# little-little-point-cloud-group/buildingSegment

Hardware: AMD Instinct MI355X
Metric: Mpoints/s segmented (kNN+normal+label) (higher is better)
Workload: dtype int32 coordinates / f64 normals; 1 GPU; urban_50m; points_per_gpu=50000000, k=16, max_nn=50, rg_mode=0, largest_plane=135921, seed_attempts=6951, fallback_queries=0, rg_rounds=25, validation_rejects=6, tie_rows=971975, parallelism=1 GPU, whole path

## Files before the change

### buildingsegment_amd/csrc/bs_knn.hip

```cpp
#include <cstdlib>
#include <type_traits>

#include "bs_common.h"
#include "bs_normal.h"

namespace bs {

namespace {

constexpr int BS_FAST_RINGS = 2;
constexpr int BS_GENERAL_RINGS = 6;

template <bool TILED>
using GridOf = std::conditional_t<TILED, TiledGridDev, GridDev>;

template <bool TILED>
__device__ inline uint64_t cell_key(uint32_t cx, uint32_t cy, uint32_t cz, uint64_t kbase)
{
  if constexpr (TILED)
    return kbase | morton_cell(cx, cy, cz);
  else
    return pack_cell(cx, cy, cz);
}

__device__ inline void tile_enter(TiledGridDev& g, int64_t s, uint64_t& kbase, int64_t& lo, int64_t& hi)
{
  const int32_t t = tile_of(g.tile_off, g.n_tiles, s);
  const TileDesc d = g.tiles[t];
#pragma unroll
  for (int a = 0; a < 3; a++) {
    g.mn[a] = d.mn[a];
    g.dim[a] = d.dim[a];
  }
  kbase = (uint64_t)t << g.mbits;
  lo = g.tile_off[t];
  hi = g.tile_off[t + 1];
}

template <bool TILED = false>
__device__ inline bool cell_lookup(const GridDev& g, uint32_t cx, uint32_t cy, uint32_t cz, int& start,
                                   int& end, uint64_t kbase = 0)
{
  const uint64_t k = cell_key<TILED>(cx, cy, cz, kbase);
  uint32_t h = hash_cell(k) & g.hmask;
  for (;;) {
    const int4 raw = *reinterpret_cast<const int4*>(&g.table[h]);
    const uint64_t ek = (uint64_t)(uint32_t)raw.x | ((uint64_t)(uint32_t)raw.y << 32);
    if (ek == k) {
      start = raw.z;
      end = raw.w;
      return true;
    }
    if (ek == ~0ull)
      return false;
    h = (h + 1) & g.hmask;
  }
}

__device__ inline bool guaranteed_radius(const GridDev& g, const int q[3], const int ci[3], int rho,
                                         uint64_t& R2)
{
  uint32_t R = 0xFFFFFFFFu;
  bool bounded = false;
#pragma unroll
  for (int a = 0; a < 3; a++) {
    if (ci[a] - rho > 0) {
      int lo = g.mn[a] + (ci[a] - rho) * g.cell;
      R = min(R, (uint32_t)(q[a] - lo + 1));
      bounded = true;
    }
    if (ci[a] + rho < g.dim[a] - 1) {
      int hi = g.mn[a] + (ci[a] + rho + 1) * g.cell - 1;
      R = min(R, (uint32_t)(hi + 1 - q[a]));
      bounded = true;
    }
  }
  R2 = (uint64_t)R * (uint64_t)R;
  return bounded;
}

__device__ inline void moments_add(Moments& m, int x, int y, int z)
{
  m.sx += x;
  m.sy += y;
  m.sz += z;
  m.sxx += (uint64_t)((int64_t)x * x);
  m.syy += (uint64_t)((int64_t)y * y);
  m.szz += (uint64_t)((int64_t)z * z);
  m.sxy += (int64_t)x * y;
  m.sxz += (int64_t)x * z;
  m.syz += (int64_t)y * z;
  m.n += 1;
}

template <int KC, bool TILED = false>
__global__ __launch_bounds__(256) void knn_fast_kernel(GridOf<TILED> g, int64_t q_begin, int64_t q_end, int K,
                                                       int max_nn, double r2, int32_t* __restrict__ neigh,
                                                       double* __restrict__ normals,
                                                       int32_t* __restrict__ fb_list,
                                                       int32_t* __restrict__ fb_count, uint64_t cert_r2,
                                                       unsigned long long* __restrict__ uncert,
                                                       int32_t* __restrict__ npos, unsigned long long* __restrict__ tie_rows)
{
  const int64_t s = xcd_logical_block() * (int64_t)blockDim.x + threadIdx.x;
  if (s >= g.n)
    return;
  const int32_t loc = g.slocal[s];
  if (loc < q_begin || loc >= q_end)
    return;
  uint64_t kbase = 0;
  if constexpr (TILED) {
    int64_t lo, hi;
    tile_enter(g, s, kbase, lo, hi);
  }
  uint64_t runner = ~0ull;
  const int4 P = g.spts[s];
  const int q[3] = {P.x, P.y, P.z};
  const int ci[3] = {(int)((uint32_t)(P.x - g.mn[0]) / (uint32_t)g.cell),
                     (int)((uint32_t)(P.y - g.mn[1]) / (uint32_t)g.cell),
                     (int)((uint32_t)(P.z - g.mn[2]) / (uint32_t)g.cell)};
  uint64_t best[KC];
  int bpos[KC];
#pragma unroll
  for (int j = 0; j < KC; j++) {
    best[j] = ~0ull;
    bpos[j] = 0;
  }
  Moments m = {};
  bool done = false;
  for (int rho = 0; rho <= BS_FAST_RINGS && !done; rho++) {
    for (int dz = -rho; dz <= rho; dz++) {
      const int cz = ci[2] + dz;
      if (cz < 0 || cz >= g.dim[2])
        continue;
      for (int dy = -rho; dy <= rho; dy++) {
        const int cy = ci[1] + dy;
        if (cy < 0 || cy >= g.dim[1])
          continue;
        const bool face = (dz == -rho || dz == rho || dy == -rho || dy == rho);
        const int step = face ? 1 : (rho > 0 ? 2 * rho : 1);
        for (int dx = -rho; dx <= rho; dx += step) {
          const int cx = ci[0] + dx;
          if (cx < 0 || cx >= g.dim[0])
            continue;
          int cs, ce;
          if (!cell_lookup<TILED>(g, (uint32_t)cx, (uint32_t)cy, (uint32_t)cz, cs, ce, kbase))
            continue;
          for (int t = cs; t < ce; t++) {
            const int4 c = g.spts[t];
            const int ex = c.x - q[0], ey = c.y - q[1], ez = c.z - q[2];
            const uint32_t d2 = (uint32_t)(ex * ex) + (uint32_t)(ey * ey) + (uint32_t)(ez * ez);
            uint64_t key = ((uint64_t)d2 << 32) | (uint32_t)c.w;
            if (key < best[KC - 1]) {
              int pay = t;
#pragma unroll
              for (int j = 0; j < KC; j++) {
                const bool lt = key < best[j];
                const uint64_t hi = lt ? best[j] : key;
                const int ph = lt ? bpos[j] : pay;
                best[j] = lt ? key : best[j];
                bpos[j] = lt ? pay : bpos[j];
                key = hi;
                pay = ph;
              }
            }
            runner = key < runner ? key : runner;
            if ((double)d2 < r2)
              moments_add(m, c.x, c.y, c.z);
          }
        }
      }
    }
    uint64_t R2;
    const bool bounded = guaranteed_radius(g, q, ci, rho, R2);
    if (!bounded) {
      done = true;
    } else {
      uint64_t kth = ~0ull;
#pragma unroll
      for (int j = 0; j < KC; j++)
        kth = (j == K - 1) ? best[j] : kth;
      const bool knn_ok = kth != ~0ull && (kth >> 32) < R2;
      const bool nrm_ok = (double)R2 >= r2;
      done = knn_ok && nrm_ok;
    }
  }
  uint64_t kth_final = ~0ull;
#pragma unroll
  for (int j = 0; j < KC; j++)
    kth_final = (j == K - 1) ? best[j] : kth_final;
  if (!done || m.n > max_nn || kth_final == ~0ull) {
    const int slot = atomicAdd(fb_count, 1);
    fb_list[slot] = (int32_t)s;
    return;
  }
  int32_t* row = neigh + (int64_t)(loc - q_begin) * K;
#pragma unroll
  for (int j = 0; j < KC; j++)
    if (j < K)
      row[j] = (int32_t)(uint32_t)best[j];
  if (npos) {
    int32_t* prow = npos + s * K;
#pragma unroll
    for (int j = 0; j < KC; j++)
      if (j < K)
        prow[j] = bpos[j];
  }
  if (normals) {
    const V3 nv = normal_from_moments(m);
    double* o = normals + 3 * (int64_t)(loc - q_begin);
    o[0] = nv.x;
    o[1] = nv.y;
    o[2] = nv.z;
    if (npos) {
      double* po = pnorm_of(npos, g.n, K) + 3 * s;
      po[0] = nv.x;
      po[1] = nv.y;
      po[2] = nv.z;
    }
  }
  if (cert_r2 && (kth_final >> 32) >= cert_r2)
    atomicAdd(uncert, 1ull);
  if (tie_rows) {
    bool tie = false;
    uint64_t next = runner;
#pragma unroll
    for (int j = 0; j + 1 < KC; j++) {
      tie = tie || (j + 1 < K && (best[j] >> 32) == (best[j + 1] >> 32));
      next = (j + 1 == K) ? best[j + 1] : next;
    }
    tie = tie || (next != ~0ull && (next >> 32) == (kth_final >> 32));
    if (tie)
      atomicAdd(tie_rows, 1ull);
  }
}

#ifndef BS_KNN_CAP4
#define BS_KNN_CAP4 0
#endif
constexpr int KBUF = 8;

template <int KC, bool REL32, bool TILED = false>
__global__ __launch_bounds__(256) __attribute__((amdgpu_waves_per_eu(KC == 16 && REL32 && BS_KNN_CAP4 ? 4 : 2))) void knn_fast2_kernel(GridOf<TILED> g, int64_t q_begin, int64_t q_end, int K,
                                                       int max_nn, double r2, int32_t* __restrict__ neigh,
                                                       double* __restrict__ normals,
                                                       int32_t* __restrict__ fb_list,
                                                       int32_t* __restrict__ fb_count, uint64_t cert_r2,
                                                       unsigned long long* __restrict__ uncert,
                                                       int32_t* __restrict__ npos, unsigned long long* __restrict__ tie_rows)
{
  const int64_t s = xcd_logical_block() * (int64_t)blockDim.x + threadIdx.x;
  if (s >= g.n)
    return;
  const int32_t loc = g.slocal[s];
  if (loc < q_begin || loc >= q_end)
    return;
  uint64_t kbase = 0;
  if constexpr (TILED) {
    int64_t lo, hi;
    tile_enter(g, s, kbase, lo, hi);
  }
  uint64_t runner = ~0ull;
  const int4 P = g.spts[s];
  const int q[3] = {P.x, P.y, P.z};
  const int ci[3] = {(int)((uint32_t)(P.x - g.mn[0]) / (uint32_t)g.cell),
                     (int)((uint32_t)(P.y - g.mn[1]) / (uint32_t)g.cell),
                     (int)((uint32_t)(P.z - g.mn[2]) / (uint32_t)g.cell)};
  __shared__ uint32_t blo[KBUF][256], bhi[KBUF][256];
  __shared__ int bps[KBUF][256];
  int nbuf = 0;
  uint64_t best[KC];
  int bpos[KC];
#pragma unroll
  for (int j = 0; j < KC; j++) {
    best[j] = ~0ull;
    bpos[j] = 0;
  }
  Moments m = {};
  int rsx = 0, rsy = 0, rsz = 0, rsxx = 0, rsyy = 0, rszz = 0, rsxy = 0, rsxz = 0, rsyz = 0, rn = 0;
  bool done = false;
  auto flush = [&]() {
    uint64_t bk[KBUF];
    int bp[KBUF];
#pragma unroll
    for (int i = 0; i < KBUF; i++) {
      const bool have = i < nbuf;
      bk[i] = have ? (((uint64_t)bhi[i][threadIdx.x] << 32) | blo[i][threadIdx.x]) : ~0ull;
      bp[i] = have ? bps[i][threadIdx.x] : 0;
    }
    nbuf = 0;
#define BS_CE(ka, pa, kb, pb)            \
  do {                                   \
    const bool sw_ = (kb) < (ka);        \
    const uint64_t tk_ = (ka);           \
    const int tp_ = (pa);                \
    (ka) = sw_ ? (kb) : (ka);            \
    (pa) = sw_ ? (pb) : (pa);            \
    (kb) = sw_ ? tk_ : (kb);             \
    (pb) = sw_ ? tp_ : (pb);             \
  } while (0)
    constexpr int net[19][2] = {{0, 1}, {2, 3}, {4, 5}, {6, 7}, {0, 2}, {1, 3}, {4, 6}, {5, 7}, {1, 2}, {5, 6},
                                {0, 4}, {3, 7}, {1, 5}, {2, 6}, {1, 4}, {3, 6}, {2, 4}, {3, 5}, {3, 4}};
#pragma unroll
    for (int c = 0; c < 19; c++)
      BS_CE(bk[net[c][0]], bp[net[c][0]], bk[net[c][1]], bp[net[c][1]]);
#pragma unroll
    for (int i = 0; i < KBUF; i++)
      BS_CE(best[KC - KBUF + i], bpos[KC - KBUF + i], bk[KBUF - 1 - i], bp[KBUF - 1 - i]);
#pragma unroll
    for (int i = 0; i < KBUF; i++)
      runner = bk[i] < runner ? bk[i] : runner;
#pragma unroll
    for (int d = KC / 2; d >= 1; d >>= 1) {
#pragma unroll
      for (int i = 0; i < KC; i++)
        if ((i & d) == 0)
          BS_CE(best[i], bpos[i], best[i + d], bpos[i + d]);
    }
#undef BS_CE
  };
  for (int rho = 0; rho <= BS_FAST_RINGS && !done; rho++) {
    for (int dz = -rho; dz <= rho; dz++) {
      const int cz = ci[2] + dz;
      if (cz < 0 || cz >= g.dim[2])
        continue;
      for (int dy = -rho; dy <= rho; dy++) {
        const int cy = ci[1] + dy;
        if (cy < 0 || cy >= g.dim[1])
          continue;
        const bool face = (dz == -rho || dz == rho || dy == -rho || dy == rho);
        const int step = face ? 1 : (rho > 0 ? 2 * rho : 1);
        for (int dx0 = -rho; dx0 <= rho; dx0 += 3 * step) {
          int4 raw[3];
          uint64_t ck[3];
          uint32_t hh[3];
          bool want[3];
#pragma unroll
          for (int u = 0; u < 3; u++) {
            const int dx = dx0 + u * step;
            const int cx = ci[0] + dx;
            want[u] = dx <= rho && cx >= 0 && cx < g.dim[0];
            ck[u] = cell_key<TILED>((uint32_t)(want[u] ? cx : ci[0]), (uint32_t)cy, (uint32_t)cz, kbase);
            hh[u] = hash_cell(ck[u]) & g.hmask;
            raw[u] = *reinterpret_cast<const int4*>(&g.table[hh[u]]);
          }
          int cs3[3], ce3[3];
#pragma unroll
          for (int u = 0; u < 3; u++) {
            cs3[u] = 0;
            ce3[u] = 0;
            if (!want[u])
              continue;
            for (;;) {
              const uint64_t ek = (uint64_t)(uint32_t)raw[u].x | ((uint64_t)(uint32_t)raw[u].y << 32);
              if (ek == ck[u]) {
                cs3[u] = raw[u].z;
                ce3[u] = raw[u].w;
                break;
              }
              if (ek == ~0ull)
                break;
              hh[u] = (hh[u] + 1) & g.hmask;
              raw[u] = *reinterpret_cast<const int4*>(&g.table[hh[u]]);
            }
          }
#pragma unroll 1
          for (int u = 0; u < 3; u++) {
            const int cs = u == 0 ? cs3[0] : (u == 1 ? cs3[1] : cs3[2]);
            const int ce = u == 0 ? ce3[0] : (u == 1 ? ce3[1] : ce3[2]);
            for (int t0 = cs; t0 < ce; t0 += 4) {
              int4 cc[4];
#pragma unroll
              for (int v = 0; v < 4; v++)
                cc[v] = g.spts[t0 + v < ce ? t0 + v : ce - 1];
#pragma unroll
              for (int v = 0; v < 4; v++) {
                const int t = t0 + v;
                const int4 c = cc[v];
                const int ex = c.x - q[0], ey = c.y - q[1], ez = c.z - q[2];
                const uint32_t d2 = (uint32_t)(ex * ex) + (uint32_t)(ey * ey) + (uint32_t)(ez * ez);
                const uint64_t key = ((uint64_t)d2 << 32) | (uint32_t)c.w;
                const bool real = t < ce;
                if (real && key < best[KC - 1]) {
                  blo[nbuf][threadIdx.x] = (uint32_t)key;
                  bhi[nbuf][threadIdx.x] = d2;
                  bps[nbuf][threadIdx.x] = t;
                  nbuf++;
                } else if (real) {
                  runner = key < runner ? key : runner;
                }
                if (__ballot(nbuf == KBUF))
                  flush();
                if (real && (double)d2 < r2) {
                  if constexpr (REL32) {
                    rsx += ex;
                    rsy += ey;
                    rsz += ez;
                    rsxx += __mul24(ex, ex);
                    rsyy += __mul24(ey, ey);
                    rszz += __mul24(ez, ez);
                    rsxy += __mul24(ex, ey);
                    rsxz += __mul24(ex, ez);
                    rsyz += __mul24(ey, ez);
                    rn += 1;
                  } else {
                    moments_add(m, c.x, c.y, c.z);
                  }
                }
              }
            }
          }
        }
      }
    }
    if (__ballot(nbuf > 0))
      flush();
    uint64_t R2;
    const bool bounded = guaranteed_radius(g, q, ci, rho, R2);
    if (!bounded) {
      done = true;
    } else {
      uint64_t kth = ~0ull;
#pragma unroll
      for (int j = 0; j < KC; j++)
        kth = (j == K - 1) ? best[j] : kth;
      const bool knn_ok = kth != ~0ull && (kth >> 32) < R2;
      const bool nrm_ok = (double)R2 >= r2;
      done = knn_ok && nrm_ok;
    }
  }
  uint64_t kth_final = ~0ull;
#pragma unroll
  for (int j = 0; j < KC; j++)
    kth_final = (j == K - 1) ? best[j] : kth_final;
  if constexpr (REL32) {
    const int64_t n64 = rn, qx = q[0], qy = q[1], qz = q[2];
    m.n = rn;
    m.sx = n64 * qx + rsx;
    m.sy = n64 * qy + rsy;
    m.sz = n64 * qz + rsz;
    m.sxx = (uint64_t)(n64 * qx * qx + 2 * qx * rsx + rsxx);
    m.syy = (uint64_t)(n64 * qy * qy + 2 * qy * rsy + rsyy);
    m.szz = (uint64_t)(n64 * qz * qz + 2 * qz * rsz + rszz);
    m.sxy = n64 * qx * qy + qx * rsy + qy * rsx + rsxy;
    m.sxz = n64 * qx * qz + qx * rsz + qz * rsx + rsxz;
    m.syz = n64 * qy * qz + qy * rsz + qz * rsy + rsyz;
  }
  if (!done || m.n > max_nn || kth_final == ~0ull) {
    const int slot = atomicAdd(fb_count, 1);
    fb_list[slot] = (int32_t)s;
    return;
  }
  int32_t* row = neigh + (int64_t)(loc - q_begin) * K;
#pragma unroll
  for (int j = 0; j < KC; j++)
    if (j < K)
      row[j] = (int32_t)(uint32_t)best[j];
  if (npos) {
    int32_t* prow = npos + s * K;
#pragma unroll
    for (int j = 0; j < KC; j++)
      if (j < K)
        prow[j] = bpos[j];
  }
  if (normals) {
    const V3 nv = normal_from_moments(m);
    double* o = normals + 3 * (int64_t)(loc - q_begin);
    o[0] = nv.x;
    o[1] = nv.y;
    o[2] = nv.z;
    if (npos) {
      double* po = pnorm_of(npos, g.n, K) + 3 * s;
      po[0] = nv.x;
      po[1] = nv.y;
      po[2] = nv.z;
    }
  }
  if (cert_r2 && (kth_final >> 32) >= cert_r2)
    atomicAdd(uncert, 1ull);
  if (tie_rows) {
    bool tie = false;
    uint64_t next = runner;
#pragma unroll
    for (int j = 0; j + 1 < KC; j++) {
      tie = tie || (j + 1 < K && (best[j] >> 32) == (best[j + 1] >> 32));
      next = (j + 1 == K) ? best[j + 1] : next;
    }
    tie = tie || (next != ~0ull && (next >> 32) == (kth_final >> 32));
    if (tie)
      atomicAdd(tie_rows, 1ull);
  }
}


__device__ inline bool cand_less(uint64_t d2a, int32_t ia, uint64_t d2b, int32_t ib)
{
  return d2a < d2b || (d2a == d2b && ia < ib);
}

__device__ inline void list_insert(uint64_t* d2s, int32_t* idxs, int32_t* poss, int& cnt, int cap, uint64_t d2, int32_t idx,
                                   int32_t pos, uint64_t* out_d2 = nullptr)
{
  int c = cnt;
  if (c == cap) {
    if (!cand_less(d2, idx, d2s[cap - 1], idxs[cap - 1])) {
      if (out_d2 && d2 < *out_d2)
        *out_d2 = d2;
      return;
    }
    if (out_d2 && d2s[cap - 1] < *out_d2)
      *out_d2 = d2s[cap - 1];
    c = cap - 1;
  }
  int j = c;
  while (j > 0 && cand_less(d2, idx, d2s[j - 1], idxs[j - 1])) {
    d2s[j] = d2s[j - 1];
    idxs[j] = idxs[j - 1];
    poss[j] = poss[j - 1];
    j--;
  }
  d2s[j] = d2;
  idxs[j] = idx;
  poss[j] = pos;
  cnt = c + 1;
}

__device__ inline void hybrid_insert(uint64_t* d2s, int32_t* gids, int32_t* poss, int& cnt, int cap,
                                     uint64_t d2, int32_t gid, int32_t pos)
{
  int c = cnt;
  if (c == cap) {
    if (!cand_less(d2, gid, d2s[cap - 1], gids[cap - 1]))
      return;
    c = cap - 1;
  }
  int j = c;
  while (j > 0 && cand_less(d2, gid, d2s[j - 1], gids[j - 1])) {
    d2s[j] = d2s[j - 1];
    gids[j] = gids[j - 1];
    poss[j] = poss[j - 1];
    j--;
  }
  d2s[j] = d2;
  gids[j] = gid;
  poss[j] = pos;
  cnt = c + 1;
}

template <bool TILED = false>
__global__ __launch_bounds__(64) void knn_general_kernel(GridOf<TILED> g, int64_t q_begin, int K, int max_nn,
                                                         double r2, int32_t* __restrict__ neigh,
                                                         double* __restrict__ normals,
                                                         const int32_t* __restrict__ fb_list,
                                                         const int32_t* __restrict__ fb_count,
                                                         uint64_t cert_r2,
                                                         unsigned long long* __restrict__ uncert,
                                                         int32_t* __restrict__ npos, unsigned long long* __restrict__ tie_rows)
{
  const int total = *fb_count;
  for (int w = blockIdx.x * blockDim.x + threadIdx.x; w < total; w += gridDim.x * blockDim.x) {
    const int32_t s = fb_list[w];
    const int32_t loc = g.slocal[s];
    uint64_t kbase = 0;
    int64_t scan_lo = 0, scan_hi = g.n;
    if constexpr (TILED)
      tile_enter(g, s, kbase, scan_lo, scan_hi);
    const int4 P = g.spts[s];
    const int q[3] = {P.x, P.y, P.z};
    const int ci[3] = {(int)((uint32_t)(P.x - g.mn[0]) / (uint32_t)g.cell),
                       (int)((uint32_t)(P.y - g.mn[1]) / (uint32_t)g.cell),
                       (int)((uint32_t)(P.z - g.mn[2]) / (uint32_t)g.cell)};
    uint64_t kd2[32], md2[64];
    int32_t kidx[32], kpos[32], mgid[64], mpos[64];
    int kc = 0, mc = 0;
    uint64_t runner = ~0ull;
    bool done = false;
    for (int rho = 0; rho <= BS_GENERAL_RINGS && !done; rho++) {
      for (int dz = -rho; dz <= rho; dz++) {
        const int cz = ci[2] + dz;
        if (cz < 0 || cz >= g.dim[2])
          continue;
        for (int dy = -rho; dy <= rho; dy++) {
          const int cy = ci[1] + dy;
          if (cy < 0 || cy >= g.dim[1])
            continue;
          const bool face = (dz == -rho || dz == rho || dy == -rho || dy == rho);
          const int step = face ? 1 : (rho > 0 ? 2 * rho : 1);
          for (int dx = -rho; dx <= rho; dx += step) {
            const int cx = ci[0] + dx;
            if (cx < 0 || cx >= g.dim[0])
              continue;
            int cs, ce;
            if (!cell_lookup<TILED>(g, (uint32_t)cx, (uint32_t)cy, (uint32_t)cz, cs, ce, kbase))
              continue;
            for (int t = cs; t < ce; t++) {
              const int4 c = g.spts[t];
              const int64_t ex = (int64_t)c.x - q[0], ey = (int64_t)c.y - q[1], ez = (int64_t)c.z - q[2];
              const uint64_t d2 = (uint64_t)(ex * ex) + (uint64_t)(ey * ey) + (uint64_t)(ez * ez);
              list_insert(kd2, kidx, kpos, kc, K, d2, c.w, t, &runner);
              if ((double)d2 < r2)
                hybrid_insert(md2, mgid, mpos, mc, max_nn, d2, c.w, t);
            }
          }
        }
      }
      uint64_t R2;
      const bool bounded = guaranteed_radius(g, q, ci, rho, R2);
      if (!bounded)
        done = true;
      else
        done = (kc == K) && (kd2[K - 1] < R2) && ((double)R2 >= r2);
    }
    if (!done) {
      kc = 0;
      mc = 0;
      runner = ~0ull;
      for (int64_t t = scan_lo; t < scan_hi; t++) {
        const int4 c = g.spts[t];
        const int64_t ex = (int64_t)c.x - q[0], ey = (int64_t)c.y - q[1], ez = (int64_t)c.z - q[2];
        const uint64_t d2 = (uint64_t)(ex * ex) + (uint64_t)(ey * ey) + (uint64_t)(ez * ez);
        list_insert(kd2, kidx, kpos, kc, K, d2, c.w, (int32_t)t, &runner);
        if ((double)d2 < r2)
          hybrid_insert(md2, mgid, mpos, mc, max_nn, d2, c.w, (int32_t)t);
      }
    }
    int32_t* row = neigh + (int64_t)(loc - q_begin) * K;
    for (int j = 0; j < K; j++)
      row[j] = kidx[j];
    if (npos)
      for (int j = 0; j < K; j++)
        npos[(int64_t)s * K + j] = kpos[j];
    if (normals) {
      Moments m = {};
      for (int j = 0; j < mc; j++) {
        const int4 c = g.spts[mpos[j]];
        moments_add(m, c.x, c.y, c.z);
      }
      const V3 nv = normal_from_moments(m);
      double* o = normals + 3 * (int64_t)(loc - q_begin);
      o[0] = nv.x;
      o[1] = nv.y;
      o[2] = nv.z;
      if (npos) {
        double* po = pnorm_of(npos, g.n, K) + 3 * (int64_t)s;
        po[0] = nv.x;
        po[1] = nv.y;
        po[2] = nv.z;
      }
    }
    if (cert_r2 && kd2[K - 1] >= cert_r2)
      atomicAdd(uncert, 1ull);
    if (tie_rows) {
      bool tie = runner == kd2[K - 1];
      for (int j = 0; j + 1 < K; j++)
        tie = tie || kd2[j] == kd2[j + 1];
      if (tie)
        atomicAdd(tie_rows, 1ull);
    }
  }
}

constexpr int GCAP = 2048;

template <bool TILED = false>
__global__ __launch_bounds__(64) void knn_general_wave_kernel(GridOf<TILED> g, int64_t q_begin, int K, int max_nn, double r2,
                                                              int32_t* __restrict__ neigh, double* __restrict__ normals,
                                                              const int32_t* __restrict__ fb_list,
                                                              const int32_t* __restrict__ fb_count, uint64_t cert_r2,
                                                              unsigned long long* __restrict__ uncert,
                                                              int32_t* __restrict__ npos, unsigned long long* __restrict__ tie_rows,
                                                              int32_t* __restrict__ fb2_list, int32_t* __restrict__ fb2_count)
{
  __shared__ uint64_t bd2[GCAP];
  __shared__ int32_t bidx[GCAP], bpos[GCAP];
  __shared__ int cxyz[64][3];
  const int lane = threadIdx.x;
  const int total = *fb_count;
  for (int w = blockIdx.x; w < total; w += gridDim.x) {
    const int32_t s = fb_list[w];
    const int32_t loc = g.slocal[s];
    uint64_t kbase = 0;
    if constexpr (TILED) {
      int64_t lo, hi;
      tile_enter(g, s, kbase, lo, hi);
    }
    const int4 P = g.spts[s];
    const int q[3] = {P.x, P.y, P.z};
    const int ci[3] = {(int)((uint32_t)(P.x - g.mn[0]) / (uint32_t)g.cell),
                       (int)((uint32_t)(P.y - g.mn[1]) / (uint32_t)g.cell),
                       (int)((uint32_t)(P.z - g.mn[2]) / (uint32_t)g.cell)};
    int count = 0;
    bool done = false, overflow = false;
    for (int rho = 0; rho <= BS_GENERAL_RINGS && !done && !overflow; rho++) {
      const int side = 2 * rho + 1, ncell = side * side * side;
      for (int c0 = 0; c0 < ncell; c0 += 64) {
        const int c = c0 + lane;
        const int dz = c / (side * side) - rho, dy = (c / side) % side - rho, dx = c % side - rho;
        const int cx = ci[0] + dx, cy = ci[1] + dy, cz = ci[2] + dz;
        const int cheb = max(max(abs(dx), abs(dy)), abs(dz));
        int cs = 0, ce = 0;
        if (c < ncell && cheb == rho && cx >= 0 && cx < g.dim[0] && cy >= 0 && cy < g.dim[1] && cz >= 0 && cz < g.dim[2]) {
          if (!cell_lookup<TILED>(g, (uint32_t)cx, (uint32_t)cy, (uint32_t)cz, cs, ce, kbase))
            cs = ce = 0;
        }
        for (int t = cs; __ballot(t < ce) != 0; t++) {
          const bool have = t < ce;
          const unsigned long long m = __ballot(have);
          const int slot = count + __popcll(m & ((1ull << lane) - 1ull));
          if (have && slot < GCAP) {
            const int4 p = g.spts[t];
            const int64_t ex = (int64_t)p.x - q[0], ey = (int64_t)p.y - q[1], ez = (int64_t)p.z - q[2];
            bd2[slot] = (uint64_t)(ex * ex) + (uint64_t)(ey * ey) + (uint64_t)(ez * ez);
            bidx[slot] = p.w;
            bpos[slot] = t;
          }
          count += __popcll(m);
        }
      }
      if (count > GCAP) {
        overflow = true;
        break;
      }
      int P2 = 64;
      while (P2 < count)
        P2 <<= 1;
      for (int i = count + lane; i < P2; i += 64) {
        bd2[i] = ~0ull;
        bidx[i] = 0x7fffffff;
        bpos[i] = 0;
      }
      __syncthreads();
      for (int k2 = 2; k2 <= P2; k2 <<= 1) {
        for (int j = k2 >> 1; j > 0; j >>= 1) {
          for (int i = lane; i < P2; i += 64) {
            const int l = i ^ j;
            if (l > i) {
              const uint64_t da = bd2[i], db = bd2[l];
              const int32_t ia = bidx[i], ib = bidx[l];
              const bool a_gt_b = da > db || (da == db && ia > ib);
              const bool up = (i & k2) == 0;
              if (a_gt_b == up) {
                bd2[i] = db;
                bd2[l] = da;
                bidx[i] = ib;
                bidx[l] = ia;
                const int32_t pa = bpos[i];
                bpos[i] = bpos[l];
                bpos[l] = pa;
              }
            }
          }
          __syncthreads();
        }
      }
      uint64_t R2;
      const bool bounded = guaranteed_radius(g, q, ci, rho, R2);
      if (!bounded)
        done = true;
      else
        done = count >= K && bd2[K - 1] < R2 && (double)R2 >= r2;
      __syncthreads();
    }
    if (overflow || !done || count < K) {
      if (lane == 0)
        fb2_list[atomicAdd(fb2_count, 1)] = s;
      __syncthreads();
      continue;
    }
    if (lane < K) {
      neigh[(int64_t)(loc - q_begin) * K + lane] = bidx[lane];
      if (npos)
        npos[(int64_t)s * K + lane] = bpos[lane];
    }
    if (normals) {
      const bool in = lane < max_nn && lane < count && (double)bd2[lane] < r2;
      const int mc = __popcll(__ballot(in));
      if (in) {
        const int4 p = g.spts[bpos[lane]];
        cxyz[lane][0] = p.x;
        cxyz[lane][1] = p.y;
        cxyz[lane][2] = p.z;
      }
      __syncthreads();
      if (lane == 0) {
        Moments m = {};
        for (int j = 0; j < mc; j++)
          moments_add(m, cxyz[j][0], cxyz[j][1], cxyz[j][2]);
        const V3 nv = normal_from_moments(m);
        double* o = normals + 3 * (int64_t)(loc - q_begin);
        o[0] = nv.x;
        o[1] = nv.y;
        o[2] = nv.z;
        if (npos) {
          double* po = pnorm_of(npos, g.n, K) + 3 * (int64_t)s;
          po[0] = nv.x;
          po[1] = nv.y;
          po[2] = nv.z;
        }
      }
    }
    if (lane == 0) {
      if (cert_r2 && bd2[K - 1] >= cert_r2)
        atomicAdd(uncert, 1ull);
      if (tie_rows) {
        bool tie = count > K && bd2[K] == bd2[K - 1];
        for (int j = 0; j + 1 < K; j++)
          tie = tie || bd2[j] == bd2[j + 1];
        if (tie)
          atomicAdd(tie_rows, 1ull);
      }
    }
    __syncthreads();
  }
}

__global__ void mark_all_kernel(GridDev g, int64_t q_begin, int64_t q_end, int32_t* fb_list,
                                int32_t* fb_count)
{
  const int64_t s = blockIdx.x * (int64_t)blockDim.x + threadIdx.x;
  if (s >= g.n)
    return;
  const int32_t loc = g.slocal[s];
  if (loc < q_begin || loc >= q_end)
    return;
  fb_list[atomicAdd(fb_count, 1)] = (int32_t)s;
}

}

template <bool TILED>
static int launch_knn(bs_ctx* ctx, const GridOf<TILED>& g, int64_t q_begin, int64_t q_end, const bs_params& p,
                      int32_t* d_neigh, double* d_normals, double cert_radius, int64_t* n_uncertified, int32_t* d_npos)
{
  hipStream_t st = ctx->stream;
  const int64_t n = g.n;
  BS_HIP(ctx, ctx->fb_list.reserve(sizeof(int32_t) * (2 * n + 32)));
  int32_t* fb_list = ctx->fb_list.as<int32_t>() + 16;
  int32_t* fb_count = ctx->fb_list.as<int32_t>();
  int32_t* fb2_list = fb_list + n + 16;
  int32_t* fb2_count = ctx->fb_list.as<int32_t>() + 2;
  unsigned long long* uncert = (unsigned long long*)(ctx->fb_list.as<int32_t>() + 4);
  unsigned long long* tie_rows = (unsigned long long*)(ctx->fb_list.as<int32_t>() + 8);
  BS_HIP(ctx, hipMemsetAsync(ctx->fb_list.p, 0, 64, st));
  const double r2 = p.radius * p.radius;
  uint64_t cert_r2 = 0;
  if (cert_radius > 0) {
    double c2 = cert_radius * cert_radius;
    cert_r2 = c2 >= 1.8e19 ? ~0ull : (uint64_t)std::ceil(c2);
    if (cert_r2 == 0)
      cert_r2 = 1;
  }
  const int blocks = (int)((n + 255) / 256);
  const int xblocks = xcd_grid(blocks);
  const bool fast_ok = (int64_t)g.cell * (2 * BS_FAST_RINGS + 1) <= 37500;
  if (fast_ok) {
    const bool buffered = getenv("BS_KNN_BUFFERED") ? atoi(getenv("BS_KNN_BUFFERED")) != 0 : true;
    const bool rel32 = r2 <= 32761.0 && !getenv("BS_KNN_MOMENTS64");
    if (buffered && p.k <= 16 && rel32)
      knn_fast2_kernel<16, true, TILED><<<xblocks, 256, 0, st>>>(g, q_begin, q_end, p.k, p.max_nn, r2, d_neigh, d_normals,
                                                         fb_list, fb_count, cert_r2, uncert, d_npos, tie_rows);
    else if (buffered && p.k <= 16)
      knn_fast2_kernel<16, false, TILED><<<xblocks, 256, 0, st>>>(g, q_begin, q_end, p.k, p.max_nn, r2, d_neigh, d_normals,
                                                          fb_list, fb_count, cert_r2, uncert, d_npos, tie_rows);
    else if (buffered && rel32)
      knn_fast2_kernel<32, true, TILED><<<xblocks, 256, 0, st>>>(g, q_begin, q_end, p.k, p.max_nn, r2, d_neigh, d_normals,
                                                         fb_list, fb_count, cert_r2, uncert, d_npos, tie_rows);
    else if (buffered)
      knn_fast2_kernel<32, false, TILED><<<xblocks, 256, 0, st>>>(g, q_begin, q_end, p.k, p.max_nn, r2, d_neigh, d_normals,
                                                          fb_list, fb_count, cert_r2, uncert, d_npos, tie_rows);
    else if (p.k <= 16)
      knn_fast_kernel<16, TILED><<<xblocks, 256, 0, st>>>(g, q_begin, q_end, p.k, p.max_nn, r2, d_neigh, d_normals,
                                                  fb_list, fb_count, cert_r2, uncert, d_npos, tie_rows);
    else
      knn_fast_kernel<32, TILED><<<xblocks, 256, 0, st>>>(g, q_begin, q_end, p.k, p.max_nn, r2, d_neigh, d_normals,
                                                  fb_list, fb_count, cert_r2, uncert, d_npos, tie_rows);
  } else {
    mark_all_kernel<<<blocks, 256, 0, st>>>(g, q_begin, q_end, fb_list, fb_count);
  }
  if (getenv("BS_KNN_GENERAL_THREAD")) {
    knn_general_kernel<TILED><<<1024, 64, 0, st>>>(g, q_begin, p.k, p.max_nn, r2, d_neigh, d_normals, fb_list, fb_count, cert_r2,
                                            uncert, d_npos, tie_rows);
  } else {
    knn_general_wave_kernel<TILED><<<8192, 64, 0, st>>>(g, q_begin, p.k, p.max_nn, r2, d_neigh, d_normals, fb_list, fb_count, cert_r2,
                                                 uncert, d_npos, tie_rows, fb2_list, fb2_count);
    knn_general_kernel<TILED><<<1024, 64, 0, st>>>(g, q_begin, p.k, p.max_nn, r2, d_neigh, d_normals, fb2_list, fb2_count, cert_r2,
                                            uncert, d_npos, tie_rows);
  }
  BS_HIP(ctx, hipGetLastError());
  int32_t hb[4];
  BS_HIP(ctx, hipMemcpyAsync(hb, ctx->fb_list.p, sizeof hb, hipMemcpyDeviceToHost, st));
  unsigned long long hu = 0, ht = 0;
  BS_HIP(ctx, hipMemcpyAsync(&hu, uncert, sizeof hu, hipMemcpyDeviceToHost, st));
  BS_HIP(ctx, hipMemcpyAsync(&ht, tie_rows, sizeof ht, hipMemcpyDeviceToHost, st));
  BS_HIP(ctx, hipStreamSynchronize(st));
  ctx->tm.n_fallback_queries = hb[0];
  ctx->tm.tie_rows = (int64_t)ht;
  if (n_uncertified)
    *n_uncertified = (int64_t)hu;
  return BS_OK;
}

int launch_knn_normals(bs_ctx* ctx, const GridDev& g, int64_t q_begin, int64_t q_end, const bs_params& p,
                       int32_t* d_neigh, double* d_normals, double cert_radius, int64_t* n_uncertified, int32_t* d_npos)
{
  return launch_knn<false>(ctx, g, q_begin, q_end, p, d_neigh, d_normals, cert_radius, n_uncertified, d_npos);
}

int launch_knn_normals_tiled(bs_ctx* ctx, const TiledGridDev& g, const bs_params& p, int32_t* d_neigh,
                             double* d_normals, int32_t* d_npos)
{
  return launch_knn<true>(ctx, g, 0, g.n, p, d_neigh, d_normals, 0.0, nullptr, d_npos);
}

}
```

Measured before the change: 200.9 Mpoints/s.

## Add phase-batched streaming kNN kernel with constant cell table as default

Adds a new kNN kernel that walks neighbour cells in fixed phases of nine using a compile-time constant offset table, ordered by ring and distance class. It resolves three hash lookups at once, stores the non-empty cell ranges in shared memory, and then streams candidate points four at a time across the ranges. It also skips cells whose minimum distance exceeds both the current k-th distance and the normal radius. The aim is better memory-level parallelism and less divergence than the per-cell loop, at the cost of more shared memory and register pressure. The new kernel becomes the default path unless BS_KNN_BUFFERED is set.

```diff
diff --git a/buildingsegment_amd/csrc/bs_knn.hip b/buildingsegment_amd/csrc/bs_knn.hip
--- a/buildingsegment_amd/csrc/bs_knn.hip
+++ b/buildingsegment_amd/csrc/bs_knn.hip
@@ -481,6 +481,331 @@
   if (tie_rows) {
     bool tie = false;
     uint64_t next = runner;
+#pragma unroll
+    for (int j = 0; j + 1 < KC; j++) {
+      tie = tie || (j + 1 < K && (best[j] >> 32) == (best[j + 1] >> 32));
+      next = (j + 1 == K) ? best[j + 1] : next;
+    }
+    tie = tie || (next != ~0ull && (next >> 32) == (kth_final >> 32));
+    if (tie)
+      atomicAdd(tie_rows, 1ull);
+  }
+}
+
+constexpr int KNN_PHASE = 9;
+constexpr int KNN_RING_CELLS(int rho) { return rho == 1 ? 27 : (2 * rho + 1) * (2 * rho + 1) * (2 * rho + 1) - (2 * rho - 1) * (2 * rho - 1) * (2 * rho - 1); }
+constexpr int KNN_RING_PHASES(int rho) { return (KNN_RING_CELLS(rho) + KNN_PHASE - 1) / KNN_PHASE; }
+constexpr int KNN_PHASES_UPTO(int rho) { return rho < 1 ? 0 : KNN_PHASES_UPTO(rho - 1) + KNN_RING_PHASES(rho); }
+constexpr int KNN_TAB = KNN_PHASES_UPTO(BS_FAST_RINGS) * KNN_PHASE;
+static_assert(BS_FAST_RINGS <= 7, "cell offsets are packed into 4 bits");
+
+struct KnnCellTab {
+  uint32_t v[KNN_TAB];
+};
+constexpr KnnCellTab knn_make_cell_tab()
+{
+  KnnCellTab t = {};
+  int n = 0;
+  for (int cls = 0; cls <= 3; cls++)
+    for (int dz = -1; dz <= 1; dz++)
+      for (int dy = -1; dy <= 1; dy++)
+        for (int dx = -1; dx <= 1; dx++)
+          if ((dx != 0) + (dy != 0) + (dz != 0) == cls)
+            t.v[n++] = (uint32_t)(dx + 8) | (uint32_t)(dy + 8) << 4 | (uint32_t)(dz + 8) << 8 | 1u << 12;
+  for (int rho = 2; rho <= BS_FAST_RINGS; rho++) {
+    for (int dz = -rho; dz <= rho; dz++)
+      for (int dy = -rho; dy <= rho; dy++)
+        for (int dx = -rho; dx <= rho; dx++)
+          if (dx == -rho || dx == rho || dy == -rho || dy == rho || dz == -rho || dz == rho)
+            t.v[n++] = (uint32_t)(dx + 8) | (uint32_t)(dy + 8) << 4 | (uint32_t)(dz + 8) << 8 | 1u << 12;
+    while (n % KNN_PHASE)
+      t.v[n++] = 8u | 8u << 4 | 8u << 8;
+  }
+  return t;
+}
+__constant__ KnnCellTab knn_cell_tab = knn_make_cell_tab();
+
+template <int KC, bool REL32, bool TILED = false>
+__global__ __launch_bounds__(256) __attribute__((amdgpu_waves_per_eu(2))) void knn_stream_kernel(GridOf<TILED> g, int64_t q_begin, int64_t q_end, int K,
+                                                       int max_nn, double r2, int32_t* __restrict__ neigh,
+                                                       double* __restrict__ normals,
+                                                       int32_t* __restrict__ fb_list,
+                                                       int32_t* __restrict__ fb_count, uint64_t cert_r2,
+                                                       unsigned long long* __restrict__ uncert,
+                                                       int32_t* __restrict__ npos, unsigned long long* __restrict__ tie_rows)
+{
+  const int64_t s = xcd_logical_block() * (int64_t)blockDim.x + threadIdx.x;
+  if (s >= g.n)
+    return;
+  const int32_t loc = g.slocal[s];
+  if (loc < q_begin || loc >= q_end)
+    return;
+  uint64_t kbase = 0;
+  if constexpr (TILED) {
+    int64_t lo, hi;
+    tile_enter(g, s, kbase, lo, hi);
+  }
+  constexpr uint32_t NONE = 0xFFFFFFFFu;
+  uint32_t runner = NONE;
+  const uint32_t r2i = r2 >= 4294967295.0 ? NONE : (uint32_t)ceil(r2);
+  const int4 P = g.spts[s];
+  const int q[3] = {P.x, P.y, P.z};
+  const int ci[3] = {(int)((uint32_t)(P.x - g.mn[0]) / (uint32_t)g.cell),
+                     (int)((uint32_t)(P.y - g.mn[1]) / (uint32_t)g.cell),
+                     (int)((uint32_t)(P.z - g.mn[2]) / (uint32_t)g.cell)};
+  int dlo[3], dhi[3];
+#pragma unroll
+  for (int a = 0; a < 3; a++) {
+    const int rel = q[a] - g.mn[a] - ci[a] * g.cell;
+    dlo[a] = rel + 1;
+    dhi[a] = g.cell - rel;
+  }
+  __shared__ uint32_t blo[KBUF][256], bhi[KBUF][256];
+  __shared__ int bps[KBUF][256];
+  __shared__ int rgs[KNN_PHASE][256], rge[KNN_PHASE][256];
+  __shared__ uint32_t rgd[KNN_PHASE][256];
+  int nbuf = 0;
+  uint64_t best[KC];
+  int bpos[KC];
+#pragma unroll
+  for (int j = 0; j < KC; j++) {
+    best[j] = ~0ull;
+    bpos[j] = 0;
+  }
+  uint32_t kd2 = NONE;
+  Moments m = {};
+  int rsx = 0, rsy = 0, rsz = 0, rsxx = 0, rsyy = 0, rszz = 0, rsxy = 0, rsxz = 0, rsyz = 0, rn = 0;
+  bool done = false;
+  auto flush = [&]() {
+    uint64_t bk[KBUF];
+    int bp[KBUF];
+#pragma unroll
+    for (int i = 0; i < KBUF; i++) {
+      const bool have = i < nbuf;
+      bk[i] = have ? (((uint64_t)bhi[i][threadIdx.x] << 32) | blo[i][threadIdx.x]) : ~0ull;
+      bp[i] = have ? bps[i][threadIdx.x] : 0;
+    }
+    nbuf = 0;
+#define BS_CE(ka, pa, kb, pb)            \
+  do {                                   \
+    const bool sw_ = (kb) < (ka);        \
+    const uint64_t tk_ = (ka);           \
+    const int tp_ = (pa);                \
+    (ka) = sw_ ? (kb) : (ka);            \
+    (pa) = sw_ ? (pb) : (pa);            \
+    (kb) = sw_ ? tk_ : (kb);             \
+    (pb) = sw_ ? tp_ : (pb);             \
+  } while (0)
+    constexpr int net[19][2] = {{0, 1}, {2, 3}, {4, 5}, {6, 7}, {0, 2}, {1, 3}, {4, 6}, {5, 7}, {1, 2}, {5, 6},
+                                {0, 4}, {3, 7}, {1, 5}, {2, 6}, {1, 4}, {3, 6}, {2, 4}, {3, 5}, {3, 4}};
+#pragma unroll
+    for (int c = 0; c < 19; c++)
+      BS_CE(bk[net[c][0]], bp[net[c][0]], bk[net[c][1]], bp[net[c][1]]);
+#pragma unroll
+    for (int i = 0; i < KBUF; i++)
+      BS_CE(best[KC - KBUF + i], bpos[KC - KBUF + i], bk[KBUF - 1 - i], bp[KBUF - 1 - i]);
+#pragma unroll
+    for (int i = 0; i < KBUF; i++)
+      runner = min(runner, (uint32_t)(bk[i] >> 32));
+#pragma unroll
+    for (int d = KC / 2; d >= 1; d >>= 1) {
+#pragma unroll
+      for (int i = 0; i < KC; i++)
+        if ((i & d) == 0)
+          BS_CE(best[i], bpos[i], best[i + d], bpos[i + d]);
+    }
+#undef BS_CE
+    kd2 = NONE;
+#pragma unroll
+    for (int j = 0; j < KC; j++)
+      kd2 = (j == K - 1) ? (uint32_t)(best[j] >> 32) : kd2;
+  };
+  int ph = 0;
+  for (int rho = 1; rho <= BS_FAST_RINGS && !done; rho++) {
+    const int ph_end = ph + KNN_RING_PHASES(rho);
+#pragma unroll 1
+    for (; ph < ph_end; ph++) {
+      int nr = 0;
+#pragma unroll 1
+      for (int c0 = 0; c0 < KNN_PHASE; c0 += 3) {
+        int4 raw[3];
+        uint64_t ck[3];
+        uint32_t hh[3], cd[3];
+        bool want[3];
+#pragma unroll
+        for (int u = 0; u < 3; u++) {
+          const uint32_t code = knn_cell_tab.v[ph * KNN_PHASE + c0 + u];
+          const int d[3] = {(int)(code & 15u) - 8, (int)((code >> 4) & 15u) - 8, (int)((code >> 8) & 15u) - 8};
+          int cc[3];
+          want[u] = (code >> 12) != 0;
+          uint32_t acc = 0;
+#pragma unroll
+          for (int a = 0; a < 3; a++) {
+            cc[a] = ci[a] + d[a];
+            want[u] = want[u] && cc[a] >= 0 && cc[a] < g.dim[a];
+            const int w = d[a] < 0 ? __mul24(-d[a] - 1, g.cell) + dlo[a] : __mul24(d[a] - 1, g.cell) + dhi[a];
+            const int w0 = d[a] == 0 ? 0 : w;
+            acc += (uint32_t)__mul24(w0, w0);
+          }
+          cd[u] = acc;
+          ck[u] = cell_key<TILED>((uint32_t)cc[0], (uint32_t)cc[1], (uint32_t)cc[2], kbase);
+          hh[u] = hash_cell(ck[u]) & g.hmask;
+          raw[u] = *reinterpret_cast<const int4*>(&g.table[hh[u]]);
+        }
+#pragma unroll
+        for (int u = 0; u < 3; u++) {
+          int cs = 0, ce = 0;
+          for (;;) {
+            const uint64_t ek = (uint64_t)(uint32_t)raw[u].x | ((uint64_t)(uint32_t)raw[u].y << 32);
+            if (ek == ck[u]) {
+              cs = want[u] ? raw[u].z : 0;
+              ce = want[u] ? raw[u].w : 0;
+              break;
+            }
+            if (ek == ~0ull)
+              break;
+            hh[u] = (hh[u] + 1) & g.hmask;
+            raw[u] = *reinterpret_cast<const int4*>(&g.table[hh[u]]);
+          }
+          if (cs < ce) {
+            rgs[nr][threadIdx.x] = cs;
+            rge[nr][threadIdx.x] = ce;
+            rgd[nr][threadIdx.x] = cd[u];
+            nr++;
+          }
+        }
+      }
+      int ri = 0, t = 0, e = 0;
+      auto pull = [&](int (&tp)[4], bool (&hv)[4]) {
+#pragma unroll
+        for (int v = 0; v < 4; v++) {
+          while (t == e && ri < nr) {
+            const uint32_t cd2 = rgd[ri][threadIdx.x];
+            const int cs = rgs[ri][threadIdx.x], ce = rge[ri][threadIdx.x];
+            ri++;
+            const bool skip = cd2 > kd2 && cd2 >= r2i;
+            t = skip ? 0 : cs;
+            e = skip ? 0 : ce;
+          }
+          hv[v] = t < e;
+          tp[v] = t;
+          t += hv[v] ? 1 : 0;
+        }
+      };
+      auto consider = [&](const int4 c, const int pos, const bool real) {
+        const int ex = c.x - q[0], ey = c.y - q[1], ez = c.z - q[2];
+        const uint32_t d2 = (uint32_t)(ex * ex) + (uint32_t)(ey * ey) + (uint32_t)(ez * ez);
+        const uint64_t key = ((uint64_t)d2 << 32) | (uint32_t)c.w;
+        if (real && key < best[KC - 1]) {
+          blo[nbuf][threadIdx.x] = (uint32_t)key;
+          bhi[nbuf][threadIdx.x] = d2;
+          bps[nbuf][threadIdx.x] = pos;
+          nbuf++;
+        } else if (real) {
+          runner = min(runner, d2);
+        }
+        if (__ballot(nbuf == KBUF))
+          flush();
+        if (real && d2 < r2i) {
+          if constexpr (REL32) {
+            rsx += ex;
+            rsy += ey;
+            rsz += ez;
+            rsxx += __mul24(ex, ex);
+            rsyy += __mul24(ey, ey);
+            rszz += __mul24(ez, ez);
+            rsxy += __mul24(ex, ey);
+            rsxz += __mul24(ex, ez);
+            rsyz += __mul24(ey, ez);
+            rn += 1;
+          } else {
+            moments_add(m, c.x, c.y, c.z);
+          }
+        }
+      };
+      for (;;) {
+        int tp[4];
+        bool hv[4];
+        pull(tp, hv);
+        if (!__ballot(hv[0]))
+          break;
+        int4 cc[4];
+#pragma unroll
+        for (int v = 0; v < 4; v++)
+          cc[v] = g.spts[hv[v] ? (int64_t)tp[v] : s];
+#pragma unroll
+        for (int v = 0; v < 4; v++)
+          consider(cc[v], tp[v], hv[v]);
+      }
+    }
+    if (__ballot(nbuf > 0))
+      flush();
+    uint64_t R2;
+    const bool bounded = guaranteed_radius(g, q, ci, rho, R2);
+    if (!bounded) {
+      done = true;
+    } else {
+      uint64_t kth = ~0ull;
+#pragma unroll
+      for (int j = 0; j < KC; j++)
+        kth = (j == K - 1) ? best[j] : kth;
+      const bool knn_ok = kth != ~0ull && (kth >> 32) < R2;
+      const bool nrm_ok = (double)R2 >= r2;
+      done = knn_ok && nrm_ok;
+    }
+  }
+  uint64_t kth_final = ~0ull;
+#pragma unroll
+  for (int j = 0; j < KC; j++)
+    kth_final = (j == K - 1) ? best[j] : kth_final;
+  if constexpr (REL32) {
+    const int64_t n64 = rn, qx = q[0], qy = q[1], qz = q[2];
+    m.n = rn;
+    m.sx = n64 * qx + rsx;
+    m.sy = n64 * qy + rsy;
+    m.sz = n64 * qz + rsz;
+    m.sxx = (uint64_t)(n64 * qx * qx + 2 * qx * rsx + rsxx);
+    m.syy = (uint64_t)(n64 * qy * qy + 2 * qy * rsy + rsyy);
+    m.szz = (uint64_t)(n64 * qz * qz + 2 * qz * rsz + rszz);
+    m.sxy = n64 * qx * qy + qx * rsy + qy * rsx + rsxy;
+    m.sxz = n64 * qx * qz + qx * rsz + qz * rsx + rsxz;
+    m.syz = n64 * qy * qz + qy * rsz + qz * rsy + rsyz;
+  }
+  if (!done || m.n > max_nn || kth_final == ~0ull) {
+    const int slot = atomicAdd(fb_count, 1);
+    fb_list[slot] = (int32_t)s;
+    return;
+  }
+  int32_t* row = neigh + (int64_t)(loc - q_begin) * K;
+#pragma unroll
+  for (int j = 0; j < KC; j++)
+    if (j < K)
+      row[j] = (int32_t)(uint32_t)best[j];
+  if (npos) {
+    int32_t* prow = npos + s * K;
+#pragma unroll
+    for (int j = 0; j < KC; j++)
+      if (j < K)
+        prow[j] = bpos[j];
+  }
+  if (normals) {
+    const V3 nv = normal_from_moments(m);
+    double* o = normals + 3 * (int64_t)(loc - q_begin);
+    o[0] = nv.x;
+    o[1] = nv.y;
+    o[2] = nv.z;
+    if (npos) {
+      double* po = pnorm_of(npos, g.n, K) + 3 * s;
+      po[0] = nv.x;
+      po[1] = nv.y;
+      po[2] = nv.z;
+    }
+  }
+  if (cert_r2 && (kth_final >> 32) >= cert_r2)
+    atomicAdd(uncert, 1ull);
+  if (tie_rows) {
+    bool tie = false;
+    uint64_t next = runner == NONE ? ~0ull : (uint64_t)runner << 32;
 #pragma unroll
     for (int j = 0; j + 1 < KC; j++) {
       tie = tie || (j + 1 < K && (best[j] >> 32) == (best[j + 1] >> 32));
@@ -854,9 +1179,22 @@
   const int xblocks = xcd_grid(blocks);
   const bool fast_ok = (int64_t)g.cell * (2 * BS_FAST_RINGS + 1) <= 37500;
   if (fast_ok) {
-    const bool buffered = getenv("BS_KNN_BUFFERED") ? atoi(getenv("BS_KNN_BUFFERED")) != 0 : true;
+    const int mode = getenv("BS_KNN_BUFFERED") ? (atoi(getenv("BS_KNN_BUFFERED")) != 0 ? 1 : 0) : 2;
+    const bool buffered = mode == 1, streams = mode == 2;
     const bool rel32 = r2 <= 32761.0 && !getenv("BS_KNN_MOMENTS64");
-    if (buffered && p.k <= 16 && rel32)
+    if (streams && p.k <= 16 && rel32)
+      knn_stream_kernel<16, true, TILED><<<xblocks, 256, 0, st>>>(g, q_begin, q_end, p.k, p.max_nn, r2, d_neigh, d_normals,
+                                                          fb_list, fb_count, cert_r2, uncert, d_npos, tie_rows);
+    else if (streams && p.k <= 16)
+      knn_stream_kernel<16, false, TILED><<<xblocks, 256, 0, st>>>(g, q_begin, q_end, p.k, p.max_nn, r2, d_neigh, d_normals,
+                                                           fb_list, fb_count, cert_r2, uncert, d_npos, tie_rows);
+    else if (streams && rel32)
+      knn_stream_kernel<32, true, TILED><<<xblocks, 256, 0, st>>>(g, q_begin, q_end, p.k, p.max_nn, r2, d_neigh, d_normals,
+                                                          fb_list, fb_count, cert_r2, uncert, d_npos, tie_rows);
+    else if (streams)
+      knn_stream_kernel<32, false, TILED><<<xblocks, 256, 0, st>>>(g, q_begin, q_end, p.k, p.max_nn, r2, d_neigh, d_normals,
+                                                           fb_list, fb_count, cert_r2, uncert, d_npos, tie_rows);
+    else if (buffered && p.k <= 16 && rel32)
       knn_fast2_kernel<16, true, TILED><<<xblocks, 256, 0, st>>>(g, q_begin, q_end, p.k, p.max_nn, r2, d_neigh, d_normals,
                                                          fb_list, fb_count, cert_r2, uncert, d_npos, tie_rows);
     else if (buffered && p.k <= 16)
```

Result: no change. 200.1 Mpoints/s (-0.4%).
